# Mamba413/bess

Measured on AMD Instinct MI355X. Metric: candidate subsets solved/sec (n=50k,p=10k,k<=200 LM), higher is better.
Workload: dtype f64; 1 GPU; configs[1]: LM sequential path, Gaussian X n=50000 p=10000, s.list=1..200, GIC, warm start, max_iter=20, is_normal; score_pass=covariance updates (cached Gram columns), collective=none, ranks_with_work=1

## Files before the change

bess_amd/csrc/bessx_k_cov.hip:

```cpp
#include "bessx_kdev.hpp"

namespace bessx {

constexpr int COV_NJ = 4;

#ifdef BESSX_PANEL_CLOCK
#define PCLK_BEGIN()                                                  \
  const unsigned long long pclk_t0_ = __builtin_amdgcn_s_memtime();   \
  const unsigned long long pclk_r0_ = __builtin_amdgcn_s_memrealtime()
#define PCLK_END(tag)                                                                                           \
  do {                                                                                                          \
    asm volatile("s_waitcnt vmcnt(0) lgkmcnt(0)" ::: "memory");                                                 \
    if (blockIdx.x == 7 && threadIdx.x == 0) {                                                                  \
      const unsigned long long dt_ = __builtin_amdgcn_s_memtime() - pclk_t0_;                                   \
      const unsigned long long dr_ = __builtin_amdgcn_s_memrealtime() - pclk_r0_;                               \
      printf("PCLK %s cycles %llu ticks100MHz %llu MHz %.0f\n", tag, dt_, dr_, dr_ ? 100.0 * (double)dt_ / (double)dr_ : 0.0); \
    }                                                                                                           \
  } while (0)
#else
#define PCLK_BEGIN()
#define PCLK_END(tag)
#endif

__device__ __forceinline__ bool cov_gate(const FitCtrl *ctrl, int slot) {
  if (ctrl->done) return false;
  if (slot == 0) return ctrl->l == 0;
  return ctrl->l == slot - 1 && !ctrl->same_prev;
}


__global__ void __launch_bounds__(256) k_cov_need(const int *__restrict__ list, int len,
                                                  const double *__restrict__ bd, double *__restrict__ bd2, int p,
                                                  int *__restrict__ slot_of, int *__restrict__ meta, int C,
                                                  int *__restrict__ fcols, FitCtrl *__restrict__ ctrl, int slot,
                                                  const int *__restrict__ A_cur, int no_restart) {
  KT(12);
  if (ctrl->done || (slot == 0 ? ctrl->l != 0 : ctrl->l != slot - 1)) return;
  cov_need_body<256>(list, len, bd, bd2, p, slot_of, meta, C, fcols, ctrl, slot, A_cur, false, no_restart != 0);
}

__global__ void __launch_bounds__(256) k_cov_fill_list(int *__restrict__ fcols, const int *__restrict__ extras,
                                                       const double *__restrict__ bd2, int *__restrict__ slot_of,
                                                       int *__restrict__ meta, FitCtrl *__restrict__ ctrl,
                                                       int parked, int spec_max, int spec, int spec_min) {
  KT(10);
  if (parked ? !ctrl->cov_stall : (ctrl->done || ctrl->l != 0)) return;
  const int nm = ctrl->cov_nmiss;
  const int tid = threadIdx.x;
  if (nm == 0) {
    if (tid == 0) ctrl->cov_nfill = 0;
    return;
  }
  const int count = meta[0];
  const int pool = spec == 2 ? 2 * COV_R : spec_max;
  const int room = spec ? min(((nm + spec_min + spec_max - 1) / spec_max) * spec_max - nm, pool) : 0;
  __shared__ int s_ne;
  if (tid < 64) {
    const int col = (spec && tid < pool) ? extras[tid] : -1;
    const double sc = col >= 0 ? bd2[col] : -1.0;
    const bool valid = col >= 0 && sc >= 0.0 && slot_of[col] < 0;
    const unsigned long long bal = __ballot(valid);
    int rank = 0;
    if (pool > spec_max) {
      for (int u = 0; u < 64; u++) {
        const double su = __shfl(sc, u);
        const int cu = __shfl(col, u);
        const bool vu = (bal >> u) & 1ull;
        if (vu && (su > sc || (su == sc && cu < col))) rank++;
      }
    } else {
      rank = __popcll(bal & ((1ull << tid) - 1ull));
    }
    if (valid && rank < room) fcols[nm + rank] = col;
    if (tid == 0) s_ne = min((int)__popcll(bal), room);
  }
  __syncthreads();
  const int tot = nm + s_ne, padded = (tot + COV_R - 1) / COV_R * COV_R;
  for (int i = tot + tid; i < padded; i += 256) fcols[i] = -1;
  for (int i = tid; i < tot; i += 256) slot_of[fcols[i]] = count + i;
  if (tid == 0) {
    meta[0] = count + tot;
    ctrl->cov_nfill = padded;
    ctrl->cov_groups += padded / COV_R;
  }
}

__global__ void __launch_bounds__(256) k_cov_publish_slots(const int *__restrict__ fcols, const int *__restrict__ slot_w,
                                                           int *__restrict__ slot_of, const FitCtrl *__restrict__ ctrl) {
  if (!ctrl->cov_stall) return;
  const int nf = ctrl->cov_nfill;
  for (int i = threadIdx.x; i < nf; i += 256) {
    const int col = fcols[i];
    if (col >= 0) slot_of[col] = slot_w[col];
  }
}

__global__ void k_cov_resume(FitCtrl *__restrict__ ctrl) {
  KT(11);
  if (ctrl->cov_stall) {
    ctrl->cov_stall = 0;
    ctrl->l = -1 - ctrl->l;
  }
}

__global__ void __launch_bounds__(256) k_cov_fill_union(const CovUnion u, int restart, const int *__restrict__ extras,
                                                        const double *__restrict__ bd2, int spec_max, int spec_min,
                                                        int *__restrict__ slot_of, int *__restrict__ meta, int p,
                                                        int *__restrict__ fcols, FitCtrl *__restrict__ fill_ctrl, int C) {
  __shared__ int wsum[4];
  __shared__ int s_ne;
  const int tid = threadIdx.x, lane = tid & 63, wave = tid >> 6;
  const int nsets = u.nf + u.dn;
  if (restart == 2) {
    int ub = 0;
    for (int f = 0; f < nsets; f++) {
      if (f < u.nf && u.on_restart[f]) continue;
      const int *__restrict__ list = f < u.nf ? u.list[f] : u.dlist[f - u.nf];
      const int len = f < u.nf ? u.len[f] : u.dlen[f - u.nf];
      for (int base = 0; base < len; base += 256) {
        const int i = base + tid;
        const int col = i < len ? list[i] : -1;
        ub += __syncthreads_count(col >= 0 && slot_of[col] < 0);
      }
    }
    restart = (meta[0] + ub + COV_R > C) ? 1 : 0;
    __syncthreads();
  }
  if (restart) {
    for (int j = tid; j < p; j += 256) slot_of[j] = -1;
    __syncthreads();
  }
  const int count = restart ? 0 : meta[0];
  int nm = 0;
  for (int f = 0; f < nsets; f++) {
    if (f < u.nf && u.on_restart[f] && !restart) continue;
    const int *__restrict__ list = f < u.nf ? u.list[f] : u.dlist[f - u.nf];
    const int len = f < u.nf ? u.len[f] : u.dlen[f - u.nf];
    for (int base = 0; base < len; base += 256) {
      const int i = base + tid;
      const int col = i < len ? list[i] : -1;
      const int miss = (col >= 0 && slot_of[col] < 0) ? 1 : 0;
      const unsigned long long bal = __ballot(miss);
      const int rank = __popcll(bal & ((1ull << lane) - 1ull));
      if (lane == 0) wsum[wave] = __popcll(bal);
      __syncthreads();
      int off = 0, tot = 0;
#pragma unroll
      for (int w = 0; w < 4; w++) {
        off += (w < wave) ? wsum[w] : 0;
        tot += wsum[w];
      }
      if (miss) {
        fcols[nm + off + rank] = col;
        slot_of[col] = count + nm + off + rank;
      }
      nm += tot;
      __syncthreads();
    }
  }
  const int room = (extras != nullptr && nm > 0) ? min(((nm + spec_min + spec_max - 1) / spec_max) * spec_max - nm, spec_max) : 0;
  if (tid == 0) s_ne = 0;
  __syncthreads();
  if (tid < 64 && room > 0) {
    const int col = tid < spec_max ? extras[tid] : -1;
    const bool valid = col >= 0 && bd2[col] >= 0.0 && slot_of[col] < 0;
    const unsigned long long bal = __ballot(valid);
    const int rank = __popcll(bal & ((1ull << tid) - 1ull));
    if (valid && rank < room) fcols[nm + rank] = col;
    if (tid == 0) s_ne = min((int)__popcll(bal), room);
  }
  __syncthreads();
  const int tot = nm + s_ne, padded = (tot + COV_R - 1) / COV_R * COV_R;
  for (int i = tot + tid; i < padded; i += 256) fcols[i] = -1;
  for (int i = nm + tid; i < tot; i += 256) slot_of[fcols[i]] = count + i;
  if (tid == 0) {
    meta[0] = count + tot;
    if (restart) {
      meta[3] += 1;
      meta[4] = 0;
    }
    fill_ctrl->cov_stall = 1;
    fill_ctrl->cov_nfill = padded;
    fill_ctrl->cov_groups += padded / COV_R;
    fill_ctrl->k_cur = count + tot;
    fill_ctrl->cov_nmiss = restart;
  }
}

#ifndef DP_PAD
#define DP_PAD 2
#endif
constexpr int DP_RB = 32;
constexpr int DP_LD = DP_RB + DP_PAD;
constexpr int DP_SC = 128;
template <bool MASKED, int NT>
__device__ __forceinline__ void cov_dp_body(const double *__restrict__ X, const double *__restrict__ aux, long ld,
                                            int p, const double *__restrict__ mask, const int *__restrict__ fcols,
                                            int g0, int rows_per_slab, int nslab, int njg,
                                            double *__restrict__ part, double *smem) {
  constexpr int NS = DP_SC / 32;
  constexpr int NL = NS + NT / 2;
  constexpr int COLS = DP_SC + 16 * NT;
  constexpr size_t BUF = (size_t)COLS * DP_LD;
  const int njg2 = (njg + 1) / 2;
  const int slab = blockIdx.x / njg2, jb = blockIdx.x - slab * njg2;
  const int tid = threadIdx.x, lane = tid & 63, wv = tid >> 6, c = lane & 15, q = lane >> 4;
  const int ru = tid & 15, cbase = tid >> 4;
  const int jc = min(jb * DP_SC + cbase, p - 1);
  const double *sx = X + (size_t)jc * ld + 2 * ru;
  const long sstride = 32 * ld;
  const int ilim = jb * DP_SC + cbase < p ? (p - 1 - (jb * DP_SC + cbase)) / 32 : 0;
  const double *src[NT / 2];
#pragma unroll
  for (int i = 0; i < NT / 2; i++) src[i] = gram_col(X, aux, ld, fcols[g0 * COV_R + i * 32 + cbase]) + 2 * ru;
  const long r_begin = (long)slab * rows_per_slab, r_end = min(r_begin + rows_per_slab, ld);
  const int nchunk = (int)((r_end - r_begin + DP_RB - 1) / DP_RB);
  d2 stA[NL], stB[NL], mA = d2{1.0, 1.0}, mB = d2{1.0, 1.0};
#define DP_LOAD1(st, ms, r, i)                                                                                  \
  do {                                                                                                          \
    if ((i) < NS)                                                                                               \
      st[i] = __builtin_nontemporal_load(reinterpret_cast<const d2 *>(sx + min((i), ilim) * sstride + (r)));    \
    else                                                                                                        \
      st[i] = *reinterpret_cast<const d2 *>(src[(i) >= NS ? (i)-NS : 0] + (r));                                 \
    if (MASKED && (i) == NL - 1) ms = *reinterpret_cast<const d2 *>(mask + (r) + 2 * ru);                       \
  } while (0)
#define DP_STORE1(buf, st, ms, i)                                                                               \
  do {                                                                                                          \
    d2 v__ = st[i];                                                                                             \
    if (MASKED && (i) >= NS) v__ = v__ * ms;                                                                    \
    *reinterpret_cast<d2 *>((buf) + 2 * ru + (size_t)((i)*32 + cbase) * DP_LD) = v__;                           \
  } while (0)
  d4 acc[NT];
#pragma unroll
  for (int t = 0; t < NT; t++) acc[t] = d4{0.0, 0.0, 0.0, 0.0};
  const size_t offa = (size_t)(wv * 16 + c) * DP_LD + 4 * q, offb = (size_t)(DP_SC + c) * DP_LD + 4 * q;
  struct Ops {
    d2 a0, a1, b0[NT], b1[NT];
  };
  auto read_ops = [&](const double *buf, int st, Ops &o) {
    o.a0 = *reinterpret_cast<const d2 *>(buf + offa + 16 * st);
    o.a1 = *reinterpret_cast<const d2 *>(buf + offa + 16 * st + 2);
#pragma unroll
    for (int t = 0; t < NT; t++) {
      o.b0[t] = *reinterpret_cast<const d2 *>(buf + offb + (size_t)t * 16 * DP_LD + 16 * st);
      o.b1[t] = *reinterpret_cast<const d2 *>(buf + offb + (size_t)t * 16 * DP_LD + 16 * st + 2);
    }
  };
#define DP_CHUNK(cur, nxt, st, ms, rload)                                                                       \
  do {                                                                                                          \
    Ops oa__, ob__;                                                                                             \
    read_ops(cur, 0, oa__);                                                                                     \
    int n__ = 0;                                                                                                \
    _Pragma("unroll") for (int s__ = 0; s__ < DP_RB / 16; s__++) {                                            \
      Ops &o__ = (s__ & 1) ? ob__ : oa__;                                                                       \
      if (s__ + 1 < DP_RB / 16) read_ops(cur, s__ + 1, (s__ & 1) ? oa__ : ob__);                                \
      __builtin_amdgcn_sched_barrier(0);                                                                        \
      _Pragma("unroll") for (int j__ = 0; j__ < 4; j__++) {                                                   \
        const double a__ = j__ == 0 ? o__.a0.x : (j__ == 1 ? o__.a0.y : (j__ == 2 ? o__.a1.x : o__.a1.y));       \
        _Pragma("unroll") for (int t__ = 0; t__ < NT; t__++) {                                                \
          const double b__ = j__ == 0 ? o__.b0[t__].x : (j__ == 1 ? o__.b0[t__].y : (j__ == 2 ? o__.b1[t__].x : o__.b1[t__].y)); \
          acc[t__] = __builtin_amdgcn_mfma_f64_16x16x4f64(a__, b__, acc[t__], 0, 0, 0);                         \
        }                                                                                                       \
                                         \
        const int due__ = (2 * NL * (s__ * 4 + j__ + 1)) / (4 * (DP_RB / 16));                                  \
        _Pragma("unroll") for (int k__ = 0; k__ < 2 * NL; k__++) {                                            \
          if (k__ >= n__ && k__ < due__) {                                                                      \
            if (k__ < NL)                                                                                       \
              DP_STORE1(nxt, st, ms, k__);                                                                      \
            else                                                                                                \
              DP_LOAD1(st, ms, rload, k__ - NL);                                                                \
          }                                                                                                     \
        }                                                                                                       \
        n__ = due__;                                                                                            \
        __builtin_amdgcn_sched_barrier(0);                                                                      \
      }                                                                                                         \
    }                                                                                                           \
  } while (0)
  double *buf0 = smem, *buf1 = smem + BUF;
  const long r_last = r_begin + (long)(nchunk - 1) * DP_RB;
#pragma unroll
  for (int i = 0; i < NL; i++) DP_LOAD1(stA, mA, r_begin, i);
#pragma unroll
  for (int i = 0; i < NL; i++) DP_STORE1(buf0, stA, mA, i);
  {
    const long r1 = min(r_begin + DP_RB, r_last), r2 = min(r_begin + 2 * DP_RB, r_last);
#pragma unroll
    for (int i = 0; i < NL; i++) DP_LOAD1(stB, mB, r1, i);
#pragma unroll
    for (int i = 0; i < NL; i++) DP_LOAD1(stA, mA, r2, i);
  }
  __syncthreads();
  for (int k = 0; k < nchunk; k += 2) {
    {
      const long rl = min(r_begin + (long)(k + 3) * DP_RB, r_last);
      DP_CHUNK(buf0, buf1, stB, mB, rl);
    }
    __syncthreads();
    if (k + 1 >= nchunk) break;
    {
      const long rl = min(r_begin + (long)(k + 4) * DP_RB, r_last);
      DP_CHUNK(buf1, buf0, stA, mA, rl);
    }
    __syncthreads();
  }
#undef DP_CHUNK
#undef DP_LOAD1
#undef DP_STORE1
  const int jg = 2 * jb + (wv >> 2);
  if (jg < njg) {
    const size_t tiles_per_slab = (size_t)njg * COV_NJ * 2;
    double *out = part + ((size_t)slab * tiles_per_slab + (size_t)(jg * COV_NJ + (wv & 3)) * 2) * 256;
    *reinterpret_cast<d4 *>(out + lane * 4) = acc[0];
    *reinterpret_cast<d4 *>(out + 256 + lane * 4) = acc[1];
    if (NT == 4) {
      double *out2 = out + (size_t)nslab * tiles_per_slab * 256;
      *reinterpret_cast<d4 *>(out2 + lane * 4) = acc[NT - 2];
      *reinterpret_cast<d4 *>(out2 + 256 + lane * 4) = acc[NT - 1];
    }
  }
}

template <bool MASKED>
__global__ void __launch_bounds__(512, 1) k_cov_panel_dp(const double *__restrict__ X, const double *__restrict__ aux,
                                                         long ld, int p, const double *__restrict__ mask,
                                                         const int *__restrict__ fcols, int g0, int ngroups,
                                                         int rows_per_slab, int nslab, int njg,
                                                         double *__restrict__ part, const FitCtrl *__restrict__ ctrl,
                                                         int big) {
  KT(5);
  if (big ? !ctrl->cov_stall : (ctrl->done || ctrl->l != 0)) return;
  const int nfill = ctrl->cov_nfill;
  if (g0 * COV_R >= nfill) return;
  extern __shared__ double smem[];
  PCLK_BEGIN();
  if (ngroups >= 2 && (g0 + 1) * COV_R < nfill)
    cov_dp_body<MASKED, 4>(X, aux, ld, p, mask, fcols, g0, rows_per_slab, nslab, njg, part, smem);
  else
    cov_dp_body<MASKED, 2>(X, aux, ld, p, mask, fcols, g0, rows_per_slab, nslab, njg, part, smem);
  PCLK_END("dp");
}

__device__ __forceinline__ void cov_reduce_body(const double *__restrict__ part, int g0, int ngroups, int nslab,
                                                int njg, int p, const int *__restrict__ fcols,
                                                const int *__restrict__ slot_of, double *__restrict__ G,
                                                const FitCtrl *__restrict__ ctrl, int big,
                                                int ex_lo, int ex_hi) {
  if (big ? !ctrl->cov_stall : (ctrl->done || ctrl->l != 0)) return;
  const int gl = blockIdx.y;
  if (gl >= ngroups || (g0 + gl) * COV_R >= ctrl->cov_nfill) return;
  const size_t tiles_per_slab = (size_t)njg * COV_NJ * 2;
  const int tile = blockIdx.x, e = threadIdx.x;
  double s = 0.0;
  for (int sl = 0; sl < nslab; sl++)
    if (sl < ex_lo || sl >= ex_hi) s += part[(((size_t)gl * nslab + sl) * tiles_per_slab + tile) * 256 + e];
  const int jt = tile >> 1, ni = tile & 1, lane = e >> 2, reg = e & 3;
  const int j = jt * 16 + (lane >> 4) + 4 * reg;
  const int ci = (g0 + gl) * COV_R + ni * 16 + (lane & 15);
  const int col = fcols[ci];
  if (j < p && col >= 0) G[(size_t)slot_of[col] * p + j] = s;
}

__global__ void __launch_bounds__(256) k_cov_reduce(const double *__restrict__ part, int g0, int ngroups, int nslab,
                                                    int njg, int p, const int *__restrict__ fcols,
                                                    const int *__restrict__ slot_of, double *__restrict__ G,
                                                    const FitCtrl *__restrict__ ctrl, int slot, int big,
                                                    int ex_lo, int ex_hi) {
  KT(6);
  cov_reduce_body(part, g0, ngroups, nslab, njg, p, fcols, slot_of, G, ctrl, big, ex_lo, ex_hi);
}

__global__ void __launch_bounds__(256) k_cov_reduce_sets(const double *__restrict__ part, int g0, int ngroups, int nslab,
                                                         int njg, int p, const int *__restrict__ fcols,
                                                         const int *__restrict__ slot_of, const CovRowSets rs,
                                                         const FitCtrl *__restrict__ ctrl, int big) {
  KT(6);
  const int r = blockIdx.z;
  cov_reduce_body(part, g0, ngroups, nslab, njg, p, fcols, slot_of, rs.G[r], ctrl, big, rs.ex_lo[r], rs.ex_hi[r]);
}

__device__ __forceinline__ void cov_compact_body(const double *__restrict__ G, int p,
                                                 const int *__restrict__ slot_of,
                                                 const int *__restrict__ fcols, int g0, double *__restrict__ GS,
                                                 int CS, const FitCtrl *__restrict__ ctrl, int big,
                                                 const double *__restrict__ xtx, int *__restrict__ meta) {
  if (big ? !ctrl->cov_stall : (ctrl->done || ctrl->l != 0)) return;
  const int gl = blockIdx.y;
  if ((g0 + gl) * COV_R >= ctrl->cov_nfill) return;
  const int j = blockIdx.x * 256 + threadIdx.x;
  const int t = j < p ? slot_of[j] : -1;
  if (t < 0) return;
  const double dj = xtx != nullptr ? xtx[j] : 0.0;
  for (int c = 0; c < COV_R; c++) {
    const int col = fcols[(g0 + gl) * COV_R + c];
    if (col < 0) continue;
    const int sc = slot_of[col];
    if (sc < 0) continue;
    const double v = G[(size_t)sc * p + j];
    if (xtx != nullptr && j != col && v * v >= (1.0 - 2e-11) * dj * xtx[col] && dj > 0.0) meta[4] = 1;
    if (sc < CS && t < CS) {
      GS[(size_t)sc * CS + t] = v;
      GS[(size_t)t * CS + sc] = v;
    }
  }
}

__global__ void __launch_bounds__(256) k_cov_compact(const double *__restrict__ G, int p,
                                                     const int *__restrict__ slot_of,
                                                     const int *__restrict__ fcols, int g0, double *__restrict__ GS,
                                                     int CS, const FitCtrl *__restrict__ ctrl, int big,
                                                     const double *__restrict__ xtx, int *__restrict__ meta) {
  KT(7);
  cov_compact_body(G, p, slot_of, fcols, g0, GS, CS, ctrl, big, xtx, meta);
}

__global__ void __launch_bounds__(256) k_cov_compact_sets(const CovRowSets rs, int p, const int *__restrict__ slot_of,
                                                          const int *__restrict__ fcols, int g0, int CS,
                                                          const FitCtrl *__restrict__ ctrl, int big,
                                                          int *__restrict__ meta) {
  KT(7);
  const int r = blockIdx.z;
  cov_compact_body(rs.G[r], p, slot_of, fcols, g0, rs.GS[r], CS, ctrl, big, rs.xtx[r], meta);
}


__device__ __forceinline__ void cov_d_body(const double *__restrict__ G, int p, const int *__restrict__ slot_of,
                                           const double *__restrict__ xty, const int *__restrict__ A_cur,
                                           const double *__restrict__ b_cur, double *__restrict__ d_out,
                                           const double *__restrict__ beta_dense, const double *__restrict__ xtx,
                                           double n_t, double lambda, const unsigned char *__restrict__ always,
                                           double *__restrict__ bd, const unsigned char *__restrict__ inA,
                                           double *__restrict__ bmm, const FitCtrl *__restrict__ ctrl, int slot,
                                           int jb ) {
  const int jj = threadIdx.x & 31, g = threadIdx.x >> 5;
  const int j = jb * 32 + jj;
  const bool epi = g == 0 && j < p;
  const double e_xty = epi ? xty[j] : 0.0, e_b = epi ? beta_dense[j] : 0.0, e_xtx = epi ? xtx[j] : 1.0;
  const unsigned char e_in = epi ? inA[j] : (unsigned char)0;
  const unsigned char e_al = (epi && always != nullptr) ? always[j] : (unsigned char)0;
  if (slot >= 0 && (ctrl->done || ctrl->l != slot - 1)) return;
  constexpr int CHUNK = 512;
  __shared__ int s_sl[CHUNK];
  __shared__ double s_b[CHUNK];
  __shared__ double sm[8][32];
  const int kc = ctrl->k_cur;
  double acc0 = 0.0, acc1 = 0.0;
  for (int base = 0; base < kc; base += CHUNK) {
    const int cnt = min(CHUNK, kc - base);
    for (int i = threadIdx.x; i < cnt; i += 256) {
      const int sl = slot_of[A_cur[base + i]];
      if (sl < 0) const_cast<FitCtrl *>(ctrl)->cov_miss = 1;
      s_sl[i] = sl;
      s_b[i] = sl < 0 ? 0.0 : b_cur[base + i];
    }
    __syncthreads();
    if (j < p) {
      for (int i0 = g; i0 < cnt; i0 += 64) {
        double gv[8], bv[8];
#pragma unroll
        for (int t = 0; t < 8; t++) {
          const int i = i0 + 8 * t;
          const bool in = i < cnt;
          gv[t] = G[(size_t)(in ? max(s_sl[i], 0) : 0) * p + j];
          bv[t] = in ? s_b[i] : 0.0;
        }
#pragma unroll
        for (int t = 0; t < 8; t += 2) {
          if (i0 + 8 * t < cnt) acc0 = fma(gv[t], bv[t], acc0);
          if (i0 + 8 * (t + 1) < cnt) acc1 = fma(gv[t + 1], bv[t + 1], acc1);
        }
      }
    }
    __syncthreads();
  }
  sm[g][jj] = acc0 + acc1;
  __syncthreads();
  if (g == 0 && j < p) {
    double t = sm[0][jj];
#pragma unroll
    for (int q = 1; q < 8; q++) t += sm[q][jj];
    const double s1 = e_xty - t;
    d_out[j] = s1;
    const double b = e_b;
    const double d = s1 / n_t - 2.0 * lambda * b;
    const double phi = sqrt(2.0 * lambda + e_xtx / n_t);
    const double inv = 1.0 / phi;
    const double tt = phi * b + inv * d;
    double v = tt * tt;
    if (e_al) v = DBL_MAX;
    bd[j] = v;
    sm[1][jj] = e_in ? v : DBL_MAX;
    sm[2][jj] = e_in ? -1.0 : v;
  } else if (g == 0) {
    sm[1][jj] = DBL_MAX;
    sm[2][jj] = -1.0;
  }
  __syncthreads();
  if (threadIdx.x == 0) {
    double mn = DBL_MAX, mx = -1.0;
    int mi = 0x7fffffff;
    for (int q = 0; q < 32; q++) {
      mn = fmin(mn, sm[1][q]);
      if (sm[2][q] > mx) {
        mx = sm[2][q];
        mi = jb * 32 + q;
      }
    }
    bmm[2 * jb] = mn;
    bmm[2 * jb + 1] = mx;
    bmm[2 * ((p + 31) / 32) + jb] = (double)mi;
    if (jb == 0) const_cast<FitCtrl *>(ctrl)->fast_same = 1;
  }
}

__global__ void __launch_bounds__(256) k_cov_d(const double *__restrict__ G, int p, const int *__restrict__ slot_of,
                                               const double *__restrict__ xty, const int *__restrict__ A_cur,
                                               const double *__restrict__ b_cur, double *__restrict__ d_out,
                                               const double *__restrict__ beta_dense, const double *__restrict__ xtx,
                                               double n_t, double lambda, const unsigned char *__restrict__ always,
                                               double *__restrict__ bd, const unsigned char *__restrict__ inA,
                                               double *__restrict__ bmm, const FitCtrl *__restrict__ ctrl, int slot) {
  KT(4);
  cov_d_body(G, p, slot_of, xty, A_cur, b_cur, d_out, beta_dense, xtx, n_t, lambda, always, bd, inA, bmm, ctrl, slot,
             blockIdx.x);
}

__global__ void __launch_bounds__(256) k_mc_cov_d(const McChain *__restrict__ chains) {
  const McChain &ch = chains[blockIdx.y];
  const int jb = blockIdx.x;
  const McState *st = ch.state;
  if (st->finished || st->parked || !st->need_d) return;
  const FitCtrl *ctrl = ch.nd.ctrl;
  if (ctrl->done || ctrl->l < 0) return;
  cov_d_body(ch.G, ch.p, ch.nd.slot_of, ch.xty, ch.nd.A_cur, ch.fz.b_cur, ch.d_out, ch.fz.beta_dense, ch.xtx, ch.n_t,
             ch.lambda, ch.always, ch.bd, ch.nd.inA, ch.bmm, ctrl, -1, jb);
}

__global__ void __launch_bounds__(256) k_cov_gram(const double *__restrict__ G, int p,
                                                  const int *__restrict__ slot_of, const int *__restrict__ A_new,
                                                  int T0, double *__restrict__ Gt, int *__restrict__ meta,
                                                  const FitCtrl *__restrict__ ctrl, int slot) {
  if (!cov_gate(ctrl, slot)) return;
  const int t = blockIdx.x, lane = threadIdx.x >> 2, r = threadIdx.x & 3;
  int I = (int)((sqrt(8.0 * (double)t + 1.0) - 1.0) * 0.5);
  while ((I + 1) * (I + 2) / 2 <= t) I++;
  while (I * (I + 1) / 2 > t) I--;
  const int J = t - I * (I + 1) / 2;
  const int a = I * 16 + (lane >> 4) + 4 * r, b = J * 16 + (lane & 15);
  double v = 0.0;
  if (a < T0 && b < T0) {
    const int sl = slot_of[A_new[b]];
    if (sl >= 0)
      v = G[(size_t)sl * p + A_new[a]];
    else
      const_cast<FitCtrl *>(ctrl)->cov_miss = 1;
  }
  Gt[(size_t)t * 256 + lane * 4 + r] = v;
}


hipError_t launch_cov_need(const int *list, int len, const double *bd, double *bd2, int p, int *slot_of, int *meta,
                           int C, int *fcols, FitCtrl *ctrl, int slot, const int *A_cur, hipStream_t st,
                           int no_restart) {
  hipLaunchKernelGGL(k_cov_need, dim3(1), dim3(256), 0, st, list, len, bd, bd2, p, slot_of, meta, C, fcols, ctrl, slot,
                     A_cur, no_restart);
  LAUNCH_CHECK();
  return hipSuccess;
}

hipError_t launch_cov_publish_slots(const int *fcols, const int *slot_w, int *slot_of, const FitCtrl *ctrl, hipStream_t st) {
  hipLaunchKernelGGL(k_cov_publish_slots, dim3(1), dim3(256), 0, st, fcols, slot_w, slot_of, ctrl);
  LAUNCH_CHECK();
  return hipSuccess;
}

hipError_t launch_cov_fill_list(int *fcols, const int *extras, const double *bd2, int *slot_of, int *meta,
                                FitCtrl *ctrl, int parked, hipStream_t st, int spec_max, int spec, int spec_min) {
  if (spec_min <= 0) spec_min = spec_max / 2;
  hipLaunchKernelGGL(k_cov_fill_list, dim3(1), dim3(256), 0, st, fcols, extras, bd2, slot_of, meta, ctrl, parked,
                     spec_max, spec, spec_min);
  LAUNCH_CHECK();
  return hipSuccess;
}

hipError_t launch_cov_resume(FitCtrl *ctrl, hipStream_t st) {
  hipLaunchKernelGGL(k_cov_resume, dim3(1), dim3(1), 0, st, ctrl);
  LAUNCH_CHECK();
  return hipSuccess;
}

hipError_t launch_cov_fill_union(const CovUnion &u, int restart, const int *extras, const double *bd2, int spec_max,
                                 int spec_min, int *slot_of, int *meta, int p, int *fcols, FitCtrl *fill_ctrl,
                                 hipStream_t st, int C) {
  if (u.nf < 1 || u.nf > 8 || u.dn < 0 || (u.dn > 0 && (!u.dlist || !u.dlen)) || spec_max > 64 || spec_min < 0 || spec_min > spec_max) return hipErrorInvalidValue;
  hipLaunchKernelGGL(k_cov_fill_union, dim3(1), dim3(256), 0, st, u, restart, extras, bd2, spec_max, spec_min, slot_of, meta, p,
                     fcols, fill_ctrl, C);
  LAUNCH_CHECK();
  return hipSuccess;
}

int cov_streamed_tiles_per_wave() { return COV_NJ; }

hipError_t launch_cov_panel(const double *X, const double *aux, long ld, int p, const double *mask, const int *fcols,
                            int g0, int ngroups, int rows_per_slab, int nslab, double *part, const FitCtrl *ctrl,
                            int parked, hipStream_t st) {
  if (ngroups < 1 || ngroups > 2) return hipErrorInvalidValue;
  const int pt = (p + 15) / 16, njg = (pt + COV_NJ - 1) / COV_NJ;
  const size_t ldsd = (size_t)2 * (DP_SC + 64) * DP_LD * sizeof(double);
  const long nbd = (long)nslab * ((njg + 1) / 2);
  if (mask)
    hipLaunchKernelGGL(k_cov_panel_dp<true>, dim3((unsigned)nbd), dim3(512), ldsd, st, X, aux, ld, p, mask, fcols, g0,
                       ngroups, rows_per_slab, nslab, njg, part, ctrl, parked);
  else
    hipLaunchKernelGGL(k_cov_panel_dp<false>, dim3((unsigned)nbd), dim3(512), ldsd, st, X, aux, ld, p, mask, fcols, g0,
                       ngroups, rows_per_slab, nslab, njg, part, ctrl, parked);
  LAUNCH_CHECK();
  return hipSuccess;
}

hipError_t cov_panel_prepare() {
  const int ldsd = (int)((size_t)2 * (DP_SC + 64) * DP_LD * sizeof(double));
  hipError_t e = hipFuncSetAttribute(reinterpret_cast<const void *>(&k_cov_panel_dp<true>),
                                     hipFuncAttributeMaxDynamicSharedMemorySize, ldsd);
  if (e != hipSuccess) return e;
  return hipFuncSetAttribute(reinterpret_cast<const void *>(&k_cov_panel_dp<false>),
                             hipFuncAttributeMaxDynamicSharedMemorySize, ldsd);
}

hipError_t launch_cov_reduce(const double *part, int p, const int *fcols, const int *slot_of, double *G, int g0,
                             int ngroups, int nslab, const FitCtrl *ctrl, int parked, hipStream_t st, int ex_lo,
                             int ex_hi) {
  const int pt = (p + 15) / 16, njg = (pt + COV_NJ - 1) / COV_NJ;
  hipLaunchKernelGGL(k_cov_reduce, dim3(njg * COV_NJ * 2, ngroups), dim3(256), 0, st, part, g0, ngroups, nslab, njg, p,
                     fcols, slot_of, G, ctrl, 0, parked, ex_lo, ex_hi);
  LAUNCH_CHECK();
  return hipSuccess;
}

hipError_t launch_cov_reduce_compact_sets(const double *part, int p, const int *fcols, const int *slot_of, int *meta,
                                          const CovRowSets &rs, int g0, int ngroups, int nslab, int CS,
                                          const FitCtrl *ctrl, int parked, hipStream_t st) {
  if (rs.nr < 1 || rs.nr > 9) return hipErrorInvalidValue;
  const int pt = (p + 15) / 16, njg = (pt + COV_NJ - 1) / COV_NJ;
  hipLaunchKernelGGL(k_cov_reduce_sets, dim3(njg * COV_NJ * 2, ngroups, rs.nr), dim3(256), 0, st, part, g0, ngroups,
                     nslab, njg, p, fcols, slot_of, rs, ctrl, parked);
  LAUNCH_CHECK();
  hipLaunchKernelGGL(k_cov_compact_sets, dim3((p + 255) / 256, ngroups, rs.nr), dim3(256), 0, st, rs, p, slot_of, fcols,
                     g0, CS, ctrl, parked, meta);
  LAUNCH_CHECK();
  return hipSuccess;
}

__global__ void __launch_bounds__(256) k_rows_permute(const double *__restrict__ X, long ld, const int *__restrict__ perm,
                                                      long ldp, double *__restrict__ Xp) {
  const long r = (long)blockIdx.x * 256 + threadIdx.x;
  if (r >= ldp) return;
  const int o = perm[r];
  Xp[(size_t)blockIdx.y * ldp + r] = o >= 0 ? X[(size_t)blockIdx.y * ld + o] : 0.0;
}
hipError_t launch_rows_permute(const double *X, long ld, int p, const int *perm, long ldp, double *Xp, hipStream_t st) {
  for (int j0 = 0; j0 < p; j0 += 32768) {
    const int nj = std::min(32768, p - j0);
    hipLaunchKernelGGL(k_rows_permute, dim3((unsigned)((ldp + 255) / 256), nj), dim3(256), 0, st, X + (size_t)j0 * ld, ld,
                       perm, ldp, Xp + (size_t)j0 * ldp);
    LAUNCH_CHECK();
  }
  return hipSuccess;
}

hipError_t launch_cov_compact(const double *G, int p, const int *slot_of, const int *fcols, int g0, int ngroups,
                              double *GS, int CS, const FitCtrl *ctrl, int parked, hipStream_t st, const double *xtx,
                              int *meta) {
  hipLaunchKernelGGL(k_cov_compact, dim3((p + 255) / 256, ngroups), dim3(256), 0, st, G, p, slot_of, fcols, g0, GS, CS,
                     ctrl, parked, xtx, meta);
  LAUNCH_CHECK();
  return hipSuccess;
}


hipError_t launch_cov_d(const double *G, int p, const int *slot_of, const double *xty, const int *A_cur,
                        const double *b_cur, double *d_out, const double *beta_dense, const double *xtx, double n_t,
                        double lambda, const unsigned char *always, double *bd, const unsigned char *inA, double *bmm,
                        const FitCtrl *ctrl, int slot, hipStream_t st) {
  hipLaunchKernelGGL(k_cov_d, dim3((p + 31) / 32), dim3(256), 0, st, G, p, slot_of, xty, A_cur, b_cur, d_out,
                     beta_dense, xtx, n_t, lambda, always, bd, inA, bmm, ctrl, slot);
  LAUNCH_CHECK();
  return hipSuccess;
}

hipError_t launch_mc_cov_d(const McChain *chains, int nchains, int p, hipStream_t st) {
  hipLaunchKernelGGL(k_mc_cov_d, dim3((p + 31) / 32, nchains), dim3(256), 0, st, chains);
  LAUNCH_CHECK();
  return hipSuccess;
}

hipError_t launch_cov_gram(const double *G, int p, const int *slot_of, const int *A_new, int T0, int mt, double *Gt,
                           int *meta, const FitCtrl *ctrl, int slot, hipStream_t st) {
  hipLaunchKernelGGL(k_cov_gram, dim3(mt * (mt + 1) / 2), dim3(256), 0, st, G, p, slot_of, A_new, T0, Gt, meta, ctrl,
                     slot);
  LAUNCH_CHECK();
  return hipSuccess;
}


}
```

Before: 18650 candidates/s.

## Retile panel DP MFMA waves into 2x2 A/B blocks with cross-chunk operand prefetch

For NT==4, each wave now computes a 2x2 block of 16x16 tiles (two A column tiles by two B tiles) instead of one A tile against four B tiles. This cuts LDS operand reads per MFMA by reusing both A and B fragments. The row loop is restructured so the next chunk's operands are read right after the barrier and the trailing barrier per chunk is dropped, overlapping LDS reads with MFMAs. The output indexing is rewritten to match the new tile assignment. wv is made wave-uniform via readfirstlane. This raises register pressure and adds risk of LDS read/write hazards from the changed barrier placement.

```diff
diff --git a/bess_amd/csrc/bessx_k_cov.hip b/bess_amd/csrc/bessx_k_cov.hip
--- a/bess_amd/csrc/bessx_k_cov.hip
+++ b/bess_amd/csrc/bessx_k_cov.hip
@@ -202,9 +202,11 @@
   constexpr int NL = NS + NT / 2;
   constexpr int COLS = DP_SC + 16 * NT;
   constexpr size_t BUF = (size_t)COLS * DP_LD;
+  constexpr int NA = NT / 2, NB = 2;
   const int njg2 = (njg + 1) / 2;
   const int slab = blockIdx.x / njg2, jb = blockIdx.x - slab * njg2;
-  const int tid = threadIdx.x, lane = tid & 63, wv = tid >> 6, c = lane & 15, q = lane >> 4;
+  const int tid = threadIdx.x, lane = tid & 63, wv = __builtin_amdgcn_readfirstlane(tid >> 6), c = lane & 15, q = lane >> 4;
+  const int ta = NT == 4 ? 2 * (wv & 3) : wv, tb = NT == 4 ? 2 * (wv >> 2) : 0;
   const int ru = tid & 15, cbase = tid >> 4;
   const int jc = min(jb * DP_SC + cbase, p - 1);
   const double *sx = X + (size_t)jc * ld + 2 * ru;
@@ -230,52 +232,65 @@
     if (MASKED && (i) >= NS) v__ = v__ * ms;                                                                    \
     *reinterpret_cast<d2 *>((buf) + 2 * ru + (size_t)((i)*32 + cbase) * DP_LD) = v__;                           \
   } while (0)
-  d4 acc[NT];
-#pragma unroll
-  for (int t = 0; t < NT; t++) acc[t] = d4{0.0, 0.0, 0.0, 0.0};
-  const size_t offa = (size_t)(wv * 16 + c) * DP_LD + 4 * q, offb = (size_t)(DP_SC + c) * DP_LD + 4 * q;
+  d4 acc[NA * NB];
+#pragma unroll
+  for (int t = 0; t < NA * NB; t++) acc[t] = d4{0.0, 0.0, 0.0, 0.0};
+  const size_t offa = (size_t)(ta * 16 + c) * DP_LD + 4 * q, offb = (size_t)(DP_SC + tb * 16 + c) * DP_LD + 4 * q;
   struct Ops {
-    d2 a0, a1, b0[NT], b1[NT];
+    d2 a0[NA], a1[NA], b0[NB], b1[NB];
   };
-  auto read_ops = [&](const double *buf, int st, Ops &o) {
-    o.a0 = *reinterpret_cast<const d2 *>(buf + offa + 16 * st);
-    o.a1 = *reinterpret_cast<const d2 *>(buf + offa + 16 * st + 2);
-#pragma unroll
-    for (int t = 0; t < NT; t++) {
-      o.b0[t] = *reinterpret_cast<const d2 *>(buf + offb + (size_t)t * 16 * DP_LD + 16 * st);
-      o.b1[t] = *reinterpret_cast<const d2 *>(buf + offb + (size_t)t * 16 * DP_LD + 16 * st + 2);
+  auto read_ops = [&](const double *rows, Ops &o) {
+#pragma unroll
+    for (int a = 0; a < NA; a++) {
+      o.a0[a] = *reinterpret_cast<const d2 *>(rows + offa + (size_t)a * 16 * DP_LD);
+      o.a1[a] = *reinterpret_cast<const d2 *>(rows + offa + (size_t)a * 16 * DP_LD + 2);
+    }
+#pragma unroll
+    for (int t = 0; t < NB; t++) {
+      o.b0[t] = *reinterpret_cast<const d2 *>(rows + offb + (size_t)t * 16 * DP_LD);
+      o.b1[t] = *reinterpret_cast<const d2 *>(rows + offb + (size_t)t * 16 * DP_LD + 2);
     }
   };
-#define DP_CHUNK(cur, nxt, st, ms, rload)                                                                       \
+#define DP_MFMA(o, j)                                                                                           \
   do {                                                                                                          \
-    Ops oa__, ob__;                                                                                             \
-    read_ops(cur, 0, oa__);                                                                                     \
-    int n__ = 0;                                                                                                \
-    _Pragma("unroll") for (int s__ = 0; s__ < DP_RB / 16; s__++) {                                            \
-      Ops &o__ = (s__ & 1) ? ob__ : oa__;                                                                       \
-      if (s__ + 1 < DP_RB / 16) read_ops(cur, s__ + 1, (s__ & 1) ? oa__ : ob__);                                \
-      __builtin_amdgcn_sched_barrier(0);                                                                        \
-      _Pragma("unroll") for (int j__ = 0; j__ < 4; j__++) {                                                   \
-        const double a__ = j__ == 0 ? o__.a0.x : (j__ == 1 ? o__.a0.y : (j__ == 2 ? o__.a1.x : o__.a1.y));       \
-        _Pragma("unroll") for (int t__ = 0; t__ < NT; t__++) {                                                \
-          const double b__ = j__ == 0 ? o__.b0[t__].x : (j__ == 1 ? o__.b0[t__].y : (j__ == 2 ? o__.b1[t__].x : o__.b1[t__].y)); \
-          acc[t__] = __builtin_amdgcn_mfma_f64_16x16x4f64(a__, b__, acc[t__], 0, 0, 0);                         \
-        }                                                                                                       \
-                                         \
-        const int due__ = (2 * NL * (s__ * 4 + j__ + 1)) / (4 * (DP_RB / 16));                                  \
-        _Pragma("unroll") for (int k__ = 0; k__ < 2 * NL; k__++) {                                            \
-          if (k__ >= n__ && k__ < due__) {                                                                      \
-            if (k__ < NL)                                                                                       \
-              DP_STORE1(nxt, st, ms, k__);                                                                      \
-            else                                                                                                \
-              DP_LOAD1(st, ms, rload, k__ - NL);                                                                \
-          }                                                                                                     \
-        }                                                                                                       \
-        n__ = due__;                                                                                            \
-        __builtin_amdgcn_sched_barrier(0);                                                                      \
+    _Pragma("unroll") for (int a__ = 0; a__ < NA; a__++) {                                                    \
+      const double av__ = (j) == 0 ? (o).a0[a__].x : ((j) == 1 ? (o).a0[a__].y : ((j) == 2 ? (o).a1[a__].x : (o).a1[a__].y)); \
+      _Pragma("unroll") for (int t__ = 0; t__ < NB; t__++) {                                                  \
+        const double bv__ = (j) == 0 ? (o).b0[t__].x : ((j) == 1 ? (o).b0[t__].y : ((j) == 2 ? (o).b1[t__].x : (o).b1[t__].y)); \
+        acc[a__ * NB + t__] = __builtin_amdgcn_mfma_f64_16x16x4f64(av__, bv__, acc[a__ * NB + t__], 0, 0, 0);   \
       }                                                                                                         \
     }                                                                                                           \
   } while (0)
+  static_assert(DP_RB == 32, "two row steps per chunk");
+#define DP_STEP(o, s, nxt, st, ms, rload)                                                                       \
+  do {                                                                                                          \
+    int n__ = (s) * NL;                                                                                         \
+    _Pragma("unroll") for (int j__ = 0; j__ < 4; j__++) {                                                     \
+      DP_MFMA(o, j__);                                                                                          \
+                                         \
+      const int due__ = (2 * NL * ((s) * 4 + j__ + 1)) / (4 * (DP_RB / 16));                                    \
+      _Pragma("unroll") for (int k__ = 0; k__ < 2 * NL; k__++) {                                              \
+        if (k__ >= n__ && k__ < due__) {                                                                        \
+          if (k__ < NL)                                                                                         \
+            DP_STORE1(nxt, st, ms, k__);                                                                        \
+          else                                                                                                  \
+            DP_LOAD1(st, ms, rload, k__ - NL);                                                                  \
+        }                                                                                                       \
+      }                                                                                                         \
+      n__ = due__;                                                                                              \
+      __builtin_amdgcn_sched_barrier(0);                                                                        \
+    }                                                                                                           \
+  } while (0)
+#define DP_CHUNK(cur, nxt, st, ms, rload)                                                                       \
+  do {                                                                                                          \
+    read_ops((cur) + 16, ob);                                                                                   \
+    __builtin_amdgcn_sched_barrier(0);                                                                          \
+    DP_STEP(oa, 0, nxt, st, ms, rload);                                                                         \
+    __syncthreads();                                                                                            \
+    read_ops(nxt, oa);                                                                                          \
+    __builtin_amdgcn_sched_barrier(0);                                                                          \
+    DP_STEP(ob, 1, nxt, st, ms, rload);                                                                         \
+  } while (0)
   double *buf0 = smem, *buf1 = smem + BUF;
   const long r_last = r_begin + (long)(nchunk - 1) * DP_RB;
 #pragma unroll
@@ -290,32 +305,34 @@
     for (int i = 0; i < NL; i++) DP_LOAD1(stA, mA, r2, i);
   }
   __syncthreads();
+  Ops oa, ob;
+  read_ops(buf0, oa);
   for (int k = 0; k < nchunk; k += 2) {
     {
       const long rl = min(r_begin + (long)(k + 3) * DP_RB, r_last);
       DP_CHUNK(buf0, buf1, stB, mB, rl);
     }
-    __syncthreads();
     if (k + 1 >= nchunk) break;
     {
       const long rl = min(r_begin + (long)(k + 4) * DP_RB, r_last);
       DP_CHUNK(buf1, buf0, stA, mA, rl);
     }
-    __syncthreads();
-  }
+  }
+#undef DP_STEP
 #undef DP_CHUNK
+#undef DP_MFMA
 #undef DP_LOAD1
 #undef DP_STORE1
-  const int jg = 2 * jb + (wv >> 2);
-  if (jg < njg) {
-    const size_t tiles_per_slab = (size_t)njg * COV_NJ * 2;
-    double *out = part + ((size_t)slab * tiles_per_slab + (size_t)(jg * COV_NJ + (wv & 3)) * 2) * 256;
-    *reinterpret_cast<d4 *>(out + lane * 4) = acc[0];
-    *reinterpret_cast<d4 *>(out + 256 + lane * 4) = acc[1];
-    if (NT == 4) {
-      double *out2 = out + (size_t)nslab * tiles_per_slab * 256;
-      *reinterpret_cast<d4 *>(out2 + lane * 4) = acc[NT - 2];
-      *reinterpret_cast<d4 *>(out2 + 256 + lane * 4) = acc[NT - 1];
+  const size_t tiles_per_slab = (size_t)njg * COV_NJ * 2;
+#pragma unroll
+  for (int a = 0; a < NA; a++) {
+    const int jg = 2 * jb + ((ta + a) >> 2);
+    if (jg < njg) {
+#pragma unroll
+      for (int t = 0; t < NB; t++) {
+        double *out = part + (((size_t)((tb + t) >> 1) * nslab + slab) * tiles_per_slab + (size_t)(jg * COV_NJ + ((ta + a) & 3)) * 2 + ((tb + t) & 1)) * 256;
+        *reinterpret_cast<d4 *>(out + lane * 4) = acc[a * NB + t];
+      }
     }
   }
 }
```

Result: faster. 19220 candidates/s, median of 6 (+3.1%).
